# gunrock/mini

Measured on AMD Instinct MI355X. Metric: MTEPS (million traversed edges/sec) BFS advance+filter, RMAT-22, higher is better.
Workload: dtype int32

## Files before the change

### include/mgx/bfs_fused.hpp

```cpp
#pragma once
#include <cstdlib>
#include <cstring>
#include <memory>

#include "runtime.hpp"
#include "env.hpp"
#include "wave.hpp"

namespace mgx {

constexpr int BFS_MAX_TRACE = 4096;
constexpr int BFS_VSHIFT = 38;
constexpr u64 BFS_EMASK = (1ull << BFS_VSHIFT) - 1ull;

struct bfs_ctrl_t {
  u64 cursor[3];
  u64 pad_a_[13];
  u64 lcursor[3];
  u64 pad_b_[13];
  u64 ledges[3];
  u64 pad_c_[13];
  u64 reached;
  u64 pad_d_[15];
  u64 merged_new;
// ... 64 lines not shown
  const int* ub_col;
  const u32* ub_col24;
  const int* ub_owner;
  u32 ub_units;
  u32 ub_units_pad;
  u32 ub_hot_only;
  const u32* ubf_col24;
  const int* ubf_owner;
  u32 ubf_units_pad;
  u32 dense_div;
  u32 vs_v[4];
  u32 vs_v9;
  u32 vs_edges;
  u32 vs_div;
  u32 vs_dummy;
  u32* flush_buf;
  u32 defer_min_marks;
  u32 defer_words;
  u32 defer_reach_mul, defer_reach_div;
  int lazy_pull;
  int merged_pull;
  u32 chain_max_edges;
  u32 chain_big_edges;
  u32 lazy_div;
  u32* slot_marks;
  const int* cold_owner;
  const int* cold_dst;
  int cold_slices;
  u32 cold_lo[BFS_COLD_MAX_SLICES];
  u32 cold_off[BFS_COLD_MAX_SLICES + 1];
// ... 793 lines not shown
  int src_plan = 1;
  int defer_words = -1;
  int defer_mul = 1, defer_div = 1;
  int do_chain = 1;
  int merged_pull = 1;
  int seed_chain = 1;
  int tail_chain = 1;
  int tail_front = 1;
  int chain_big = -1;
  int cold = 1;
  int lazy = -1;
  long long defer = -1;
  int spin = -1;
  int build_list = 0;
  int mini = 1;
  int batch_overlap = 1;
  int many_spare = 0;
#ifdef MGX_LAB
  int flags = 0;
  int build_diag = 0;
  int dense_diag = 0;
#endif
  static bfs_run_opts_t from_env() {
    bfs_run_opts_t o;
    auto geti = [](const char* name, int& out) { if (const char* e = mgx::env(name)) out = atoi(e); };
    auto getll = [](const char* name, long long& out) { if (const char* e = mgx::env(name)) out = atoll(e); };
    geti("MGX_BFS_COLD_TEST", o.cold_test);
    geti("MGX_BFS_MERGED_PUSH", o.merged);
    geti("MGX_BFS_DENSE", o.dense);
    geti("MGX_BFS_VSHORT", o.vshort);
// ... 7 lines not shown
    geti("MGX_BFS_HOT_UNITS", o.hot_units);
    geti("MGX_BFS_COLD", o.cold);
    if (const char* e = mgx::env("MGX_BFS_DEFER_REACH")) {
      o.defer_mul = atoi(e);
      const char* sl = strchr(e, '/');
      o.defer_div = sl ? atoi(sl + 1) : 1;
      if (o.defer_div < 1) o.defer_div = 1;
    }
    geti("MGX_BFS_SEED_CHAIN", o.seed_chain);
    geti("MGX_BFS_MERGED_PULL", o.merged_pull);
    geti("MGX_BFS_DO_CHAIN", o.do_chain);
    geti("MGX_BFS_TAIL_CHAIN", o.tail_chain);
    geti("MGX_BFS_TAIL_FRONT", o.tail_front);
    geti("MGX_BFS_CHAIN_BIG_EDGES", o.chain_big);
    geti("MGX_BFS_MINI", o.mini);
    geti("MGX_BFS_BATCH_OVERLAP", o.batch_overlap);
    if (o.many_spare < 0) o.many_spare = 0;
    geti("MGX_BFS_LAZY", o.lazy);
    if (o.lazy > (1 << 20)) o.lazy = 1 << 20;
#ifdef MGX_LAB
    geti("MGX_BFS_FLAGS", o.flags);
    geti("MGX_BFS_BUILD_DIAG", o.build_diag);
    geti("MGX_BFS_DENSE_DIAG", o.dense_diag);
#else
#endif
    return o;
  }
};

struct bfs_alt_state_t {
// ... 108 lines not shown
```

### include/mgx/bfs_fused_mini.hpp

```cpp
#pragma once
#include "bfs_fused.hpp"
#include "bfs_fused_chain.hpp"

namespace mgx {

constexpr int BFS_MINI_WGS = 64;
constexpr int BFS_MINI_LCAP = 4096;
constexpr int BFS_MINI_WCAP = 8192;
constexpr u32 BFS_MINI_EDGES_LATE = 131072;
constexpr u32 BFS_MINI_EDGES_EARLY = 32768;
constexpr u32 BFS_MINI_SHORT_ROWS = 65536;
constexpr size_t bfs_mini_lds_bytes() {
  return (size_t)(2 * BFS_MINI_LCAP + 4) * 4 + (size_t)BFS_MINI_WCAP * 4 + 64 * 8 + 256;
}

__device__ __forceinline__ bool bfs_level_is_mini(const bfs_fused_args_t& a, const bfs_ctrl_t* c, int slot) {
  if (a.mode != 0 || c->lazy_slot == slot) return false;
  const u64 cur = c->cursor[slot % 3], lcur = c->lcursor[slot % 3];
  const u64 E = (cur & BFS_EMASK) + c->ledges[slot % 3];
  const bool late = c->reached * 4ull >= (u64)(u32)a.n;
  return (lcur >> BFS_VSHIFT) <= (u64)BFS_MINI_LCAP && (cur >> BFS_VSHIFT) <= (u64)BFS_MINI_SHORT_ROWS &&
         E <= (u64)(late ? BFS_MINI_EDGES_LATE : BFS_MINI_EDGES_EARLY);
}

template <int NT>
__device__ __forceinline__ void bfs_mini_body(const bfs_fused_args_t& a, int arg, u32 blk, u32 nblk) {
  constexpr int NW = NT / WAVE;
  constexpr u64 CNT1 = 1ull << 40;
  constexpr u64 DEGMASK = CNT1 - 1ull;
  extern __shared__ __attribute__((aligned(16))) char smem[];
  u32* const s_loff = (u32*)smem;
  u32* const s_lrow = s_loff + BFS_MINI_LCAP + 4;
  u32* const s_win = s_lrow + BFS_MINI_LCAP;
  u64* const s_scan = (u64*)(s_win + BFS_MINI_WCAP);
  __shared__ int s_cnt, s_maxdeg;
  __shared__ u64 s_base[2];
  __shared__ u32 s_long_true;
  bfs_ctrl_t* const c = a.ctrl;
  int slot, level;
  bfs_resolve(c, arg, slot, level);
  if (c->done) return;
  const u64 cur = c->cursor[slot % 3], lcur = c->lcursor[slot % 3];
  const u64 ledges = c->ledges[slot % 3];
  const int nf_s = (int)(cur >> BFS_VSHIFT), nf_l = (int)(lcur >> BFS_VSHIFT);
  const u32 Es = (u32)(cur & BFS_EMASK), Rl = (u32)(lcur & BFS_EMASK);
  const int in = slot & 1, out = (slot + 1) & 1;
  const bool first_thread = blk == 0 && threadIdx.x == 0;
  if (nf_s + nf_l == 0) {
    if (first_thread) {
      c->cursor[(slot + 2) % 3] = 0; c->lcursor[(slot + 2) % 3] = 0; c->ledges[(slot + 2) % 3] = 0;
// ... 37 lines not shown
    c->sum_long_vertices += (u64)nf_l;
    c->push_levels += 1;
    c->small_levels += 1;
    c->mini_slots += 1;
    c->slots += 1;
    c->slot_level[(slot + 1) & 3] = level + 1;
    c->flush_count[(slot + 1) & 1] = 0;
    bfs_slot_marks_clear(a, slot + 1);
    c->fb_slot = -1;
  }
  const int lane = lane_id();
  const int wave = threadIdx.x / WAVE;
  const u32 long_min = a.long_min > 0 ? (u32)a.long_min : 0xFFFFFFFFu;
  const int new_label = level + 1;
  for (int i = threadIdx.x; i < nf_l; i += NT) { s_loff[i] = a.lq_off[in][i]; s_lrow[i] = a.lq_row[in][i]; }
  if (threadIdx.x == 0) { s_loff[nf_l] = Rl; s_cnt = 0; s_maxdeg = 0; }
  __syncthreads();

  u64* const cur_s = &c->cursor[(slot + 1) % 3];
  u64* const cur_l = &c->lcursor[(slot + 1) % 3];
  u32* __restrict__ const out_row_s = a.fr_row[out];
  u32* __restrict__ const out_off_s = a.fr_off[out];
  u32* __restrict__ const out_row_l = a.lq_row[out];
  u32* __restrict__ const out_off_l = a.lq_off[out];
  int found = 0;

  auto flush = [&]() {
    __syncthreads();
    const int W = s_cnt;
    for (int first = 0; first < W; first += NT) {
      const int i = first + (int)threadIdx.x;
// ... 20 lines not shown
        if (tot_l >> 40) atomicAdd(&c->ledges[(slot + 1) % 3], (u64)s_long_true);
      }
      __syncthreads();
      if (deg) {
        const u64 b = is_long ? s_base[1] : s_base[0];
        const u64 at = is_long ? ex_l : ex_s;
        const u64 pos = (b >> BFS_VSHIFT) + (at >> 40);
        (is_long ? out_row_l : out_row_s)[pos] = ro;
        (is_long ? out_off_l : out_off_s)[pos] = (u32)((b & BFS_EMASK) + (at & DEGMASK)) | (is_long ? (deg & 63u) : 0u);
      }
      __syncthreads();
    }
    if (threadIdx.x == 0) s_cnt = 0;
    __syncthreads();
  };
  auto visit = [&](bool act, u32 d) {
    bool win = false;
    if (act) {
      const u32 bit = 1u << (d & 31u);
      const u32 seen = a.visited[d >> 5];
      if (!(seen & bit)) win = !(atomicOr(a.visited + (d >> 5), bit) & bit);
    }
    const u64 bal = __ballot(win);
    if (bal) {
      int at = 0;
      if (lane == 0) at = atomicAdd(&s_cnt, __popcll(bal));
      at = __builtin_amdgcn_readfirstlane(at);
      if (win) { s_win[at + rank_in_mask(bal)] = d; ++found; }
    }
  };

  {
    const u32 U = Rl >> 6;
    const u32 Wt = nblk * NW, w0 = blk * NW + (u32)wave;
    const u32 iters = (U + Wt - 1u) / Wt;
    for (u32 t = 0; t < iters; ++t) {
      const u32 u = w0 + t * Wt;
      bool act = false;
      u32 d = 0;
      if (u < U) {
        const u32 r0 = u << 6;
        int lo = 0, hi = nf_l;
        while (hi - lo > 1) { const int mid = (lo + hi) >> 1; if ((s_loff[mid] & ~63u) <= r0) lo = mid; else hi = mid; }
        const u32 e0 = s_loff[lo];
        const u32 deg = bfs_lq_degree(e0, s_loff[lo + 1]);
        const u32 rank = r0 - (e0 & ~63u) + (u32)lane;
        act = rank < deg;
        if (act) d = (u32)a.col_indices[s_lrow[lo] + rank];
      }
      visit(act, d);
      __syncthreads();
      const int cnt_now = s_cnt;
      __syncthreads();
      if (cnt_now > BFS_MINI_WCAP - NT) flush();
    }
  }
  if (nf_s > 0 && (u64)Es >= 4ull * (u64)nf_s) {
    const u32* __restrict__ fr_row = a.fr_row[in];
    const u32* __restrict__ fr_off = a.fr_off[in];
    const u32 iters = (Es + (u32)gthreads - 1u) / (u32)gthreads;
    for (u32 t = 0; t < iters; ++t) {
      const u64 r64 = (u64)gtid + (u64)t * (u64)gthreads;
      const bool act = r64 < (u64)Es;
      const u32 r = act ? (u32)r64 : 0u;
      int lo = 0, hi = nf_s;
      while (hi - lo > 1) { const int mid = (lo + hi) >> 1; if (fr_off[mid] <= r) lo = mid; else hi = mid; }
      const u32 d = act ? (u32)a.col_indices[fr_row[lo] + (r - fr_off[lo])] : 0u;
      visit(act, d);
      __syncthreads();
      const int cnt_now = s_cnt;
      __syncthreads();
      if (cnt_now > BFS_MINI_WCAP - NT) flush();
    }
  } else
  {
    const u32* __restrict__ fr_row = a.fr_row[in];
    const u32* __restrict__ fr_off = a.fr_off[in];
    const u32 iters = ((u32)nf_s + (u32)gthreads - 1u) / (u32)gthreads;
    for (u32 t = 0; t < iters; ++t) {
      const long long i = gtid + (long long)t * gthreads;
      u32 row = 0, deg = 0;
      if (i < nf_s) {
        const u32 e0 = fr_off[i], e1 = (i + 1 < nf_s) ? fr_off[i + 1] : Es;
        row = fr_row[i];
        deg = e1 - e0;
      }
      int wmax = (int)deg;
#pragma unroll
      for (int sh = WAVE / 2; sh > 0; sh >>= 1) { const int o = __shfl_xor(wmax, sh, WAVE); wmax = o > wmax ? o : wmax; }
      if (lane == 0 && wmax) atomicMax(&s_maxdeg, wmax);
      __syncthreads();
      const u32 kmax = (u32)s_maxdeg;
      for (u32 k = 0; k < kmax; ++k) {
        const bool act = k < deg;
        const u32 d = act ? (u32)a.col_indices[row + k] : 0u;
        visit(act, d);
        __syncthreads();
        const int cnt_now = s_cnt;
        __syncthreads();
        if (cnt_now > BFS_MINI_WCAP - NT) flush();
      }
      __syncthreads();
      if (threadIdx.x == 0) s_maxdeg = 0;
      __syncthreads();
    }
  }
  flush();
  found = (int)wave_sum((u32)found);
  if (lane == 0 && found) atomicAdd(&c->reached_mini, (u64)found);
}
template <int NT>
__global__ __launch_bounds__(NT) void k_bfs_mini(bfs_fused_args_t a, int arg) {
  bfs_mini_body<NT>(a, arg, blockIdx.x, gridDim.x);
}

}
```

### include/mgx/bfs_fused_run.hpp

```cpp
#pragma once
#include <cassert>
#include <cstring>
#include <vector>
#include <unistd.h>
#include "bfs_fused.hpp"
#include "bfs_fused_chain.hpp"
#include "bfs_fused_cold.hpp"
#include "bfs_fused_dense.hpp"
#include "bfs_fused_mini.hpp"
#include "bfs_fused_pull.hpp"
#include "bfs_fused_stream.hpp"
#include "bfs_fused_vshort.hpp"
#include "bfs_fused_sparse.hpp"
#include "bfs_fused_wave.hpp"
#include "row_layout.hpp"

namespace mgx {

struct bfs_layout_t {
  const int* row_offsets = nullptr;
  const int* col_indices = nullptr;
  const int* new_of_old = nullptr;
  const int* old_of_new = nullptr;
  const row_layout_t* rows = nullptr;
// ... 108 lines not shown
  if (c->lazy_slot == slot) return;
  if (!bfs_level_is_chained(a, cur, lcur, c->ledges[slot % 3], a.chain_big_edges, BFS_CHAIN_CAP_BIG)) return;
  bfs_chain_body<1024, true, BFS_CHAIN_CAP_BIG>(a, slot, level);
}
__global__ __launch_bounds__(1024) void k_bfs_chain_inplace(bfs_fused_args_t a, int arg) {
  bfs_chain_inplace_body(a, arg);
}

struct bfs_seam_init_t {
  long long nwords;
  const bfs_ctrl_t* prev_ctrl;
  bfs_ctrl_t* prev_head;
  int src, head_words;
};
static_assert(2 * sizeof(bfs_fused_args_t) + sizeof(bfs_seam_init_t) + 64 <= 4096, "a seam launch's two argument structs fit the 4 KB of kernel arguments");
__global__ __launch_bounds__(1024) void k_bfs_seam_mini_init(bfs_fused_args_t a, int arg_a, bfs_fused_args_t b, bfs_seam_init_t init) {
  if (blockIdx.x < (u32)BFS_MINI_WGS) bfs_mini_body<1024>(a, arg_a, blockIdx.x, (u32)BFS_MINI_WGS);
  else bfs_init_body<1024>(b, init.src, init.nwords, init.prev_ctrl, init.prev_head, init.head_words, blockIdx.x - (u32)BFS_MINI_WGS,
                           gridDim.x - (u32)BFS_MINI_WGS);
}
__global__ __launch_bounds__(1024) void k_bfs_seam_chain_chain(bfs_fused_args_t a, int arg_a, bfs_fused_args_t b, int arg_b) {
  if (blockIdx.x == 0) bfs_chain_inplace_body(a, arg_a);
  else bfs_chain_inplace_body(b, arg_b);
}
__global__ __launch_bounds__(1024) void k_bfs_seam_chain_init(bfs_fused_args_t a, int arg_a, bfs_fused_args_t b, bfs_seam_init_t init) {
  if (blockIdx.x == 0) bfs_chain_inplace_body(a, arg_a);
  else bfs_init_body<1024>(b, init.src, init.nwords, init.prev_ctrl, init.prev_head, init.head_words, blockIdx.x - 1u, gridDim.x - 1u);
}

#ifdef MGX_LAB
__global__ __launch_bounds__(1024, 8) void k_bfs_push_stream_diag(bfs_fused_args_t a, int arg) {
  const bfs_slot_plan_t p = bfs_slot_plan(a, arg);
  if (p.empty || p.chained) return;
  bfs_stream_body<1024, BFS_STREAM_HOTW2, 8, false, true, true>(a, p.slot, blockIdx.x, gridDim.x, p.level);
// ... 74 lines not shown
inline void bfs_launch_push(const bfs_fused_args_t& a, int level, standard_context_t& ctx, int open_here, bool coldt, u32 grid_div = 1) {
  if (grid_div < 1u) grid_div = 1u;
  u32 per = (u32)ctx.num_cus * 2 / grid_div;
  if (per < 32u) per = 32u;
  const u32 nstream = a.long_min > 0 ? per : 0u;
  const u32 nwave = per;
  const u32 ncold = a.cold_dst ? a.cold_wgs[a.cold_slices] : 0u;
  if (coldt) hipLaunchKernelGGL(k_bfs_push_level<true>, dim3(ncold + nstream + nwave), dim3(1024), bfs_push_lds_bytes(), ctx.stream(), a, level, nstream, open_here, ncold);
  else hipLaunchKernelGGL(k_bfs_push_level<false>, dim3(ncold + nstream + nwave), dim3(1024), bfs_push_lds_bytes(), ctx.stream(), a, level, nstream, open_here, ncold);
}

struct bfs_launch_plan_t {
  bfs_fused_args_t a;
  bool coldt = false, build2_ok = false;
  bool minis = false;
  u32 nstream = 0, nwave = 0, ncold = 0;
  int lab_flags = 0;
  long long nwords = 0;
  int mode = 0;
  int* labels = nullptr;
};

inline bfs_launch_plan_t bfs_fused_plan(bfs_fused_state_t& st, const int* row_offsets, const int* col_indices, int* labels,
                                        standard_context_t& ctx, const bfs_layout_t* layout, int mode, float alpha,
                                        const int* in_offsets, const int* in_indices) {
  bfs_launch_plan_t plan;
  bfs_fused_args_t& a = plan.a;
  const bfs_run_opts_t& opt = st.opts;
  const bool relabelled = layout && layout->row_offsets;
  static const row_layout_t no_rows;
// ... 51 lines not shown
    a.ub_col24 = R.ubh.col24.data(); a.ub_owner = R.ubh.owner.data();
    a.ub_units = (u32)R.ubh.units; a.ub_units_pad = (u32)R.ubh.units_pad;
  }
  a.ub_hot_only = hot_units ? 1u : 0u;
  a.ubf_col24 = hot_units ? R.ub.col24.data() : nullptr; a.ubf_owner = hot_units ? R.ub.owner.data() : nullptr;
  a.ubf_units_pad = hot_units ? (u32)R.ub.units_pad : 0u;
  const bool packed = units && st.opts.pack24 && (R.ub.col24.data() != nullptr || hot_units);
  a.dense_div = !units ? 0u : (opt.dense >= 0 ? (u32)opt.dense : (packed ? 8u : st.dense_div));
  const bool vs = relabelled && R.vs_dummy != 0 && R.vs_long_min == st.long_min && st.long_min > 0 && !coldt && !lab_flags &&
                  R.vs_edges > 0;
  for (int i = 0; i < 4; ++i) a.vs_v[i] = vs ? R.vs_v[i] : 0u;
  a.vs_v9 = (vs && R.vs_v9 >= R.vs_v[1] && R.vs_v9 <= R.vs_v[2]) ? R.vs_v9 : (vs ? R.vs_v[2] : 0u);
  a.vs_edges = vs ? R.vs_edges : 0u;
  a.vs_dummy = vs ? R.vs_dummy : 0u;
  a.vs_div = !vs ? 0u : (opt.vshort >= 0 ? (u32)opt.vshort : st.vshort_div);
#ifdef MGX_LAB
  a.dense_diag = opt.dense_diag;
  a.build_diag = opt.build_diag;
#endif
  if (!st.slot_marks.size()) st.slot_marks = mem_t<u32>((size_t)2 * BFS_MARK_CTRS * BFS_MARK_STRIDE, ctx);
  a.slot_marks = st.slot_marks.data();
  a.merged_pull = (mode == 1 && opt.merged_pull && opt.merged && !lab_flags) ? 1 : 0;
  const long long defer = opt.defer >= 0 ? opt.defer : (long long)st.defer_min_marks;
  if (defer > 0 && !lab_flags && !st.flush_buf.size()) st.flush_buf = mem_t<u32>((size_t)BFS_FLUSH_MAX * BFS_FLUSH_WORDS, ctx);
  a.flush_buf = (defer > 0 && !lab_flags) ? st.flush_buf.data() : nullptr;
  a.defer_min_marks = (u32)defer;
  {
    int dw = opt.defer_words >= 0 ? opt.defer_words : BFS_FLUSH_WORDS;
    if (dw > BFS_FLUSH_WORDS) dw = BFS_FLUSH_WORDS;
    a.defer_words = (u32)(dw / 32 * 32);
// ... 14 lines not shown
  for (int i = 0; i <= BFS_COLD_MAX_SLICES; ++i) a.cold_cb[i] = cold_pk ? R.cold_cb[i] : 0u;
  for (int i = 0; i < BFS_COLD_MAX_SLICES; ++i) a.cold_lo[i] = cold ? R.cold_lo[i] : 0u;
  for (int i = 0; i <= BFS_COLD_MAX_SLICES; ++i) { a.cold_off[i] = cold ? R.cold_off[i] : 0u; a.cold_wgs[i] = cold ? R.cold_wgs[i] : 0u; }
  const bool colds = cold && a.vs_div && R.colds_pairs > 0 && R.colds_dst.data() && opt.cold != 2;
  a.colds_owner = colds ? R.colds_owner.data() : nullptr;
  a.colds_dst = colds ? R.colds_dst.data() : nullptr;
  for (int i = 0; i <= BFS_COLD_MAX_SLICES; ++i) a.colds_off[i] = colds ? R.colds_off[i] : 0u;
  const size_t cold_words = cold ? (size_t)R.cold_wgs[R.cold_slices] * BFS_COLD_WORDS : 0;
  if (cold && st.cold_flush.size() < cold_words) { ctx.synchronize(); st.cold_flush = mem_t<u32>(cold_words, ctx); }
  a.cold_flush = cold ? st.cold_flush.data() : nullptr;
  a.lazy_pull = (mode == 1 && build2_ok && !opt.build_list && opt.lazy != 0) ? 1 : 0;
  a.lazy_div = (a.dense_div && a.vs_div && build2_ok && !opt.build_list && !a.cold_all) ? (opt.lazy >= 0 ? (u32)opt.lazy : st.lazy_div) : 0u;
  plan.coldt = coldt;
  plan.build2_ok = build2_ok;
  plan.minis = mode == 0 && opt.mini != 0 && a.chain_big_edges != 0u && opt.merged && !lab_flags && (st.n >= (1 << 22) || opt.mini == 2);
  plan.nstream = a.long_min > 0 ? (u32)ctx.num_cus * 2 : 0u;
  plan.nwave = (u32)ctx.num_cus * 2;
  plan.ncold = (!coldt && a.cold_dst) ? a.cold_wgs[a.cold_slices] : 0u;
  plan.lab_flags = lab_flags;
  plan.nwords = nwords;
  plan.mode = mode;
  plan.labels = labels;
  return plan;
}

inline bool bfs_wants_src_shapes(const bfs_fused_state_t& st, int mode) {
  return mode == 0 && st.opts.src_plan && st.opts.tail_chain && st.opts.mini != 0 && st.opts.merged && st.opts.seed_chain &&
         (st.n >= (1 << 22) || st.opts.mini == 2);
}
inline int bfs_classify_source(const bfs_fused_state_t& st, const bfs_launch_plan_t& plan, const bfs_layout_t* layout, int src, int idx = 0) {
// ... 3 lines not shown
  const unsigned* const sh = layout->src_shapes + (size_t)idx * 4;
  const u64 deg = sh[0], e1 = sh[1], s1 = sh[2], l1 = sh[3];
  if (deg == 0 || e1 == 0xFFFFFFFFull) return BFS_SRC_UNKNOWN;
  if ((1ull + s1 + l1) * 4ull >= (u64)(u32)a.n) return BFS_SRC_UNKNOWN;
  const u64 lim = a.chain_big_edges < BFS_CHAIN_EARLY_EDGES ? a.chain_big_edges : BFS_CHAIN_EARLY_EDGES;
  const u64 chain_cap = lim < (u64)BFS_CHAIN_CAP_BIG ? lim : (u64)BFS_CHAIN_CAP_BIG;
  u64 E, rs, rl;
  if (deg > chain_cap) {
    const bool is_long = a.long_min > 0 && deg >= (u64)a.long_min;
    E = deg; rs = is_long ? 0 : 1; rl = is_long ? 1 : 0;
  } else if (e1 > chain_cap) {
    E = e1; rs = s1; rl = l1;
  } else {
    return BFS_SRC_UNKNOWN;
  }
  const bool mini = rl <= (u64)BFS_MINI_LCAP && rs <= (u64)BFS_MINI_SHORT_ROWS && E <= (u64)BFS_MINI_EDGES_EARLY;
  return mini ? BFS_SRC_ABSORB : BFS_SRC_SKIP;
}
inline int bfs_class_slots(const bfs_fused_state_t& st, int cls) {
  if (cls == BFS_SRC_UNKNOWN) return st.slots_hint;
  if (st.cls_at[cls] > 0) return st.cls_max[cls];
  if (cls == BFS_SRC_SKIP && st.cls_at[BFS_SRC_ABSORB] > 0) return st.cls_max[BFS_SRC_ABSORB] + 1 > st.slots_hint ? st.cls_max[BFS_SRC_ABSORB] + 1 : st.slots_hint;
  return st.slots_hint;
}

inline void bfs_enqueue_chain_inplace(const bfs_launch_plan_t& plan, int slot, hipStream_t s) {
  hipLaunchKernelGGL(k_bfs_chain_inplace, dim3(1), dim3(1024), bfs_chain_lds_bytes(BFS_CHAIN_CAP_BIG), s, plan.a, bfs_slot_arg(slot));
}
inline void bfs_enqueue_mini(const bfs_launch_plan_t& plan, int slot, hipStream_t s) {
  hipLaunchKernelGGL(k_bfs_mini<1024>, dim3(BFS_MINI_WGS), dim3(1024), bfs_mini_lds_bytes(), s, plan.a, bfs_slot_arg(slot));
}
inline int bfs_enqueue_start(const bfs_fused_state_t& st, const bfs_launch_plan_t& plan, int src, standard_context_t& ctx,
                             const bfs_ctrl_t* prev_ctrl = nullptr, bfs_ctrl_t* prev_head = nullptr, int head_words = 0,
                             bool front_mini = true) {
  hipStream_t s = ctx.stream();
  hipLaunchKernelGGL(k_bfs_fused_init, dim3(grid_for(((long long)st.n + 3) / 4, BLOCK, ctx.num_cus * 8)), dim3(BLOCK), 0, s, plan.a, src,
                     plan.nwords, prev_ctrl, prev_head, head_words);
  if (plan.a.chain_big_edges) bfs_enqueue_chain_inplace(plan, 0, s);
  if (plan.minis && front_mini) { bfs_enqueue_mini(plan, 0, s); return 1; }
  return 0;
}
inline bool bfs_fused_plan_alt(bfs_fused_state_t& st, const bfs_launch_plan_t& plan, standard_context_t& ctx, bfs_launch_plan_t& p) {
  if (!st.alt && !st.alt_refused) {
    st.alt = bfs_alt_state_t::make(st.n, st.bitmap_words(), ctx);
    st.alt_refused = !st.alt;
// ... 13 lines not shown
  a.ctrl = t.ctrl;
  a.slot_marks = t.slot_marks;
  return true;
}
inline void bfs_enqueue_seam(const bfs_fused_state_t& st, const bfs_launch_plan_t& plan_a, const bfs_launch_plan_t& tail_a, int sl_a,
                             const bfs_launch_plan_t& plan_b, int src, bfs_ctrl_t* prev_head, int head_words, standard_context_t& ctx) {
  hipStream_t s = ctx.stream();
  bfs_seam_init_t init;
  init.nwords = plan_b.nwords;
  init.prev_ctrl = plan_b.a.ctrl;
  init.prev_head = prev_head;
  init.src = src;
  init.head_words = head_words;
  const int want = grid_for(((long long)st.n + 3) / 4, 1024, 1 << 20);
  if (plan_a.minis) {
    int ninit = ctx.num_cus - BFS_MINI_WGS;
    if (ninit < 64) ninit = 64;
    if (ninit > want) ninit = want;
    hipLaunchKernelGGL(k_bfs_seam_mini_init, dim3(BFS_MINI_WGS + ninit), dim3(1024), bfs_mini_lds_bytes(), s, plan_a.a, bfs_slot_arg(sl_a),
                       plan_b.a, init);
    hipLaunchKernelGGL(k_bfs_seam_chain_chain, dim3(2), dim3(1024), bfs_chain_lds_bytes(BFS_CHAIN_CAP_BIG), s, tail_a.a, bfs_slot_arg(sl_a + 1),
                       plan_b.a, bfs_slot_arg(0));
  } else {
    int ninit = ctx.num_cus - 1;
    if (ninit < 16) ninit = 16;
    if (ninit > want) ninit = want;
    hipLaunchKernelGGL(k_bfs_seam_chain_init, dim3(1 + ninit), dim3(1024), bfs_chain_lds_bytes(BFS_CHAIN_CAP_BIG), s, tail_a.a, bfs_slot_arg(sl_a),
                       plan_b.a, init);
    bfs_enqueue_chain_inplace(plan_b, 0, s);
  }
}
inline void bfs_enqueue_build(const bfs_fused_state_t& st, const bfs_launch_plan_t& plan, int arg, hipStream_t s) {
  if (st.opts.build_list || !plan.build2_ok)
    hipLaunchKernelGGL((k_bfs_build<512, true>), dim3(bfs_build_grid(st.n, 512)), dim3(512), 0, s, plan.a, arg,
                       (const u32*)nullptr, plan.labels, st.n, 1, 0, 1);
// ... 17 lines not shown
  st.tail_from = 1 << 30;
  if (!(a.chain_big_edges && st.opts.tail_chain)) return;
  const int lv = hc->levels < trace_avail ? hc->levels : trace_avail;
  int kind[64];
  const int L = lv < 64 ? lv : 64;
  bool pulled = false;
  u64 reached = 1;
  int extra_big = lv > 64 ? lv - 64 : 0;
  (void)extra_big;
  for (int l = 0; l < L; ++l) {
    const u64 t = hc->trace[l];
    if (l > 0) reached += t >> BFS_VSHIFT;
    const bool late = reached * 4ull >= (u64)(u32)a.n;
    const u64 lim = late || a.chain_big_edges < BFS_CHAIN_EARLY_EDGES ? a.chain_big_edges : BFS_CHAIN_EARLY_EDGES;
    bool small = (t >> BFS_VSHIFT) <= (u64)BFS_CHAIN_CAP_BIG && (t & BFS_EMASK) <= lim;
    bool mid = (t >> BFS_VSHIFT) <= (u64)BFS_MINI_SHORT_ROWS && (t & BFS_EMASK) <= (u64)(late ? BFS_MINI_EDGES_LATE : BFS_MINI_EDGES_EARLY);
    if (mode == 1) {
      const float unvisited = (float)((long long)a.n - (long long)reached);
      if (unvisited < (float)(long long)(t >> BFS_VSHIFT) * a.alpha) pulled = true;
      if (pulled) small = false;
      mid = false;
    }
    kind[l] = small ? 0 : (minis && mid ? 1 : 2);
  }
  auto slots_needed = [&](bool front_mini) {
    int lo = 0, hi = L;
    while (lo < hi && kind[lo] == 0) ++lo;
    if (minis && front_mini && lo < hi && kind[lo] == 1) ++lo;
    while (hi > lo && kind[hi - 1] == 0) --hi;
    if (minis && hi > lo && kind[hi - 1] == 1) {
      --hi;
// ... 64 lines not shown
          else
#endif
          bfs_launch_push_part<2>(a, arg, ctx, coldt, nstream + ncold, nstream);
        }
        if (timed) MGX_HIP(hipEventRecord(st.wev[3 * i + 1], s));
        bfs_launch_push_part<3>(a, arg, ctx, coldt, nwave, 0);
        if (timed) MGX_HIP(hipEventRecord(st.wev[3 * i + 2], s));
      } else {
        bfs_launch_push_part<0>(a, arg, ctx, coldt, nstream + ncold + nwave, nstream);
      }
      if (mode == 1 && !a.merged_pull)
        hipLaunchKernelGGL(k_bfs_pull_level<256>, dim3(ctx.num_cus * 8), dim3(256), 0, s, a, arg);
      bfs_enqueue_build(st, plan, arg, s);
      if (timed_merged) MGX_HIP(hipEventRecord(st.wev[3 * i + 2], s));
    }
    if (plan.minis && batch == 0) { bfs_enqueue_mini(plan, slot, s); ++slot; }
    if (a.chain_big_edges && (slot >= st.tail_from || plan.minis) && opt.tail_chain) chain_inplace(slot);
    if (batch_events) MGX_HIP(hipEventRecord(st.ev1, s));
    constexpr size_t head_bytes = offsetof(bfs_ctrl_t, trace) + 64 * sizeof(u64);
    if ((opt.spin >= 0 ? opt.spin != 0 : st.spin) && !batch_events) {
      const u64 seq = ++st.seq;
      hipLaunchKernelGGL(k_bfs_publish, dim3(1), dim3(256), 0, s, (const bfs_ctrl_t*)st.ctrl.data(), st.host_ctrl.data(), st.host_seq.data(), seq,
                         (int)(head_bytes / 4));
      MGX_CHECK_LAUNCH("fused BFS: kernel launch");
      volatile u64* const flag = st.host_seq.data();
      long long spins = 0;
      while (*flag != seq) {
        if (++spins > 20000000LL) { MGX_HIP(hipStreamSynchronize(s)); break; }
        __builtin_ia32_pause();
      }
      __atomic_thread_fence(__ATOMIC_ACQUIRE);
// ... 106 lines not shown
    const bfs_launch_plan_t& P = plans[me];
    bfs_ctrl_t* const prev_head = pending[me] >= 0 ? bfs_many_head(heads, pending[me]) : (bfs_ctrl_t*)nullptr;
    pending[me] = i;
    int sl;
    if (i == 0 || state_of(i - 1) == me) {
      sl = bfs_enqueue_start(st, P, srcs[i], ctx, prev_head ? P.a.ctrl : (const bfs_ctrl_t*)nullptr, prev_head, head_words, cls != BFS_SRC_SKIP);
    } else {
      const int sl_a = plan.minis ? last_slots[(size_t)i - 1] - 1 : last_slots[(size_t)i - 1];
      bfs_enqueue_seam(st, plans[me ^ 1], tails[me ^ 1], sl_a, P, srcs[i], prev_head, head_words, ctx);
      sl = 0;
      if (plan.minis && cls != BFS_SRC_SKIP) { bfs_enqueue_mini(P, 0, s); sl = 1; }
    }
    for (int k = 0; k < my_slots; ++k, ++sl) bfs_enqueue_slot(st, P, sl, ctx);
    if (overlap && i + 1 == lead && !st.alt) second_state();
    const bool seam_behind = i + 1 < count && state_of(i + 1) != me;
    if (plan.minis) { if (!seam_behind) bfs_enqueue_mini(P, sl, s); ++sl; }
    if (tail && !seam_behind) bfs_enqueue_chain_inplace(tails[me], sl, s);
    last_slots[(size_t)i] = sl;
    classes[(size_t)i] = cls;
  }
  tail_guard.release();
  const u64 seq = ++st.seq;
  assert(pending[0] == count - 1);
  if (pending[1] >= 0)
    hipLaunchKernelGGL(k_bfs_publish2, dim3(1), dim3(256), 0, s, (const bfs_ctrl_t*)plans[0].a.ctrl, bfs_many_head(heads, pending[0]),
                       (const bfs_ctrl_t*)plans[1].a.ctrl, bfs_many_head(heads, pending[1]), st.host_seq.data(), seq, head_words);
  else
    hipLaunchKernelGGL(k_bfs_publish, dim3(1), dim3(256), 0, s, (const bfs_ctrl_t*)st.ctrl.data(), bfs_many_head(heads, count - 1), st.host_seq.data(), seq, head_words);
  MGX_CHECK_LAUNCH("fused BFS (batch of sources): kernel launch");
  {
    volatile u64* const flag = st.host_seq.data();
// ... 31 lines not shown
```

### include/mgx/env.hpp

```cpp
#pragma once
#include <cstdio>
#include <cstdlib>
#include <cstring>

namespace mgx {

struct env_switch_t { const char* name; const char* what; };

inline const env_switch_t* env_switches(int* count) {
  static const env_switch_t table[] = {
    {"MGX_BFS_DENSE", "0 / N: unit-block body for long rows off / a level takes it from frontier edges >= units / N"},
    {"MGX_BFS_VSHORT", "0 / N: short rows vertex by vertex off / threshold divisor"},
    {"MGX_BFS_LAZY", "0 / N: lazy queues off / the build writes no queues behind a push that stored >= n / N marks"},
    {"MGX_BFS_COLD", "0 / 2 (lab: 1): cold-edge pass off / on"},
    {"MGX_BFS_COLD_LISTS", "0 / 1 (lab: 2): whether the layout builds the long rows' cold-edge lists"},
    {"MGX_BFS_COLD_PACK", "0: keep the 8-byte cold pairs instead of the packed 4-byte ones"},
    {"MGX_BFS_COLD_TEST", "0 / 1: bitmap probe of cold neighbours off / on (default: by graph size)"},
    {"MGX_BFS_FLAT_LISTS", "0: a flat graph keeps the ordinary layout instead of all-entry pair lists"},
    {"MGX_BFS_HOT_UNITS", "0: no second copy of the unit blocks without the cold lists' entries"},
    {"MGX_BFS_PACK24", "0: 32-bit unit-block entries instead of the 24-bit copy"},
    {"MGX_BFS_MINI", "0 / 2: no M launches / M launches on every graph (default: from 2^22 vertices on)"},
    {"MGX_BFS_BATCH_OVERLAP", "0: a batch of sources runs in one traversal state, no launch shared by two traversals"},
    {"MGX_BFS_SEED_CHAIN", "0: the chain of small levels at the start runs inside slot 0's push launch"},
    {"MGX_BFS_TAIL_CHAIN", "0: no in-place chain launch behind the last slots"},
    {"MGX_BFS_TAIL_FRONT", "0: no chain in front of the last slots"},
    {"MGX_BFS_CHAIN_BIG_EDGES", "largest level an in-place chain launch runs (edges)"},
    {"MGX_BFS_CHAIN_MAX_EDGES", "largest level block 0 runs inside the push launch (0: no chains)"},
    {"MGX_BFS_MERGED_PUSH", "0: the parts of a slot's push as separate launches"},
    {"MGX_BFS_MERGED_PULL", "0: direction-optimising runs: the bottom-up sweep as a launch of its own"},
    {"MGX_BFS_DO_CHAIN", "0: direction-optimising runs: no chains of small top-down levels"},
    {"MGX_BFS_DEFER", "0 / N: deferred hot marks off / a workgroup flushes its bitmap above N claims"},
    {"MGX_BFS_DEFER_REACH", "\"mul/div\": a level defers its hot marks while reached * mul < range * div"},
    {"MGX_BFS_DEFER_WORDS", "words of the bitmap prefix whose marks are deferred (default: all)"},
    {"MGX_BFS_BUILD_LIST", "1: the list-based queue build of round 1"},
    {"MGX_BFS_SRC_PLAN", "0: no per-source launch plan"},
    {"MGX_BFS_LONG_MIN", "long-row threshold of the layout (entries)"},
// ... 58 lines not shown
```

Baseline: 462,700.

## Widen mini BFS launch for late levels and restage short-row expansion in LDS

Adds a late-level rule that sends levels behind the peak with up to a configurable edge count (default 1M) into the mini kernel. When it applies, the tail launch and the seam init launch are sized to the CU count instead of 64 workgroups. The short-row expansion now gives each workgroup a contiguous edge share and stages the row offsets in LDS in chunks, replacing the per-thread global binary search and the degree-max loop. It also halves the window capacity, drops per-iteration barriers in favour of periodic flushes, and issues relaxed atomic loads with batched visited reads. This trades possible lost occupancy or imbalance for fewer launches and less synchronisation on tail levels.

```diff
diff --git a/include/mgx/bfs_fused.hpp b/include/mgx/bfs_fused.hpp
--- a/include/mgx/bfs_fused.hpp
+++ b/include/mgx/bfs_fused.hpp
@@ -102,6 +102,7 @@
   u32 vs_edges;
   u32 vs_div;
   u32 vs_dummy;
+  u32 mini_late_edges;
   u32* flush_buf;
   u32 defer_min_marks;
   u32 defer_words;
@@ -925,6 +926,7 @@
   int spin = -1;
   int build_list = 0;
   int mini = 1;
+  int mini_late_edges = -1;
   int batch_overlap = 1;
   int many_spare = 0;
 #ifdef MGX_LAB
@@ -962,6 +964,7 @@
     geti("MGX_BFS_TAIL_FRONT", o.tail_front);
     geti("MGX_BFS_CHAIN_BIG_EDGES", o.chain_big);
     geti("MGX_BFS_MINI", o.mini);
+    geti("MGX_BFS_MINI_LATE_EDGES", o.mini_late_edges);
     geti("MGX_BFS_BATCH_OVERLAP", o.batch_overlap);
     if (o.many_spare < 0) o.many_spare = 0;
     geti("MGX_BFS_LAZY", o.lazy);
diff --git a/include/mgx/bfs_fused_mini.hpp b/include/mgx/bfs_fused_mini.hpp
--- a/include/mgx/bfs_fused_mini.hpp
+++ b/include/mgx/bfs_fused_mini.hpp
@@ -6,21 +6,39 @@
 
 constexpr int BFS_MINI_WGS = 64;
 constexpr int BFS_MINI_LCAP = 4096;
-constexpr int BFS_MINI_WCAP = 8192;
+constexpr int BFS_MINI_WCAP = 4096;
 constexpr u32 BFS_MINI_EDGES_LATE = 131072;
 constexpr u32 BFS_MINI_EDGES_EARLY = 32768;
 constexpr u32 BFS_MINI_SHORT_ROWS = 65536;
+constexpr u32 BFS_MINI_LATE_EDGES_DEFAULT = 1u << 20;
+constexpr u32 BFS_MINI_LATE_FINDS = 131072;
 constexpr size_t bfs_mini_lds_bytes() {
   return (size_t)(2 * BFS_MINI_LCAP + 4) * 4 + (size_t)BFS_MINI_WCAP * 4 + 64 * 8 + 256;
+}
+static_assert(bfs_mini_lds_bytes() <= 64 * 1024, "an init workgroup fits beside an M workgroup on a CU");
+
+__host__ __device__ constexpr bool bfs_mini_takes(u64 rows_s, u64 rows_l, u64 E, u64 reached, u32 n, u32 vs3, u32 late_edges) {
+  if (rows_l > (u64)BFS_MINI_LCAP) return false;
+  const bool late = reached * 4ull >= (u64)n;
+  if (!late) return rows_s <= (u64)BFS_MINI_SHORT_ROWS && E <= (u64)BFS_MINI_EDGES_EARLY;
+  if (vs3 == 0u || late_edges <= BFS_MINI_EDGES_LATE) return rows_s <= (u64)BFS_MINI_SHORT_ROWS && E <= (u64)BFS_MINI_EDGES_LATE;
+  const u64 finds = (u64)vs3 > reached ? (u64)vs3 - reached : 0ull;
+  return E <= (u64)late_edges && finds <= (u64)BFS_MINI_LATE_FINDS;
+}
+inline int bfs_mini_tail_wgs(u32 late_edges, int num_cus) {
+  if (late_edges <= BFS_MINI_EDGES_LATE) return BFS_MINI_WGS;
+  return num_cus > 0 ? num_cus : 1;
 }
 
 __device__ __forceinline__ bool bfs_level_is_mini(const bfs_fused_args_t& a, const bfs_ctrl_t* c, int slot) {
   if (a.mode != 0 || c->lazy_slot == slot) return false;
   const u64 cur = c->cursor[slot % 3], lcur = c->lcursor[slot % 3];
   const u64 E = (cur & BFS_EMASK) + c->ledges[slot % 3];
-  const bool late = c->reached * 4ull >= (u64)(u32)a.n;
-  return (lcur >> BFS_VSHIFT) <= (u64)BFS_MINI_LCAP && (cur >> BFS_VSHIFT) <= (u64)BFS_MINI_SHORT_ROWS &&
-         E <= (u64)(late ? BFS_MINI_EDGES_LATE : BFS_MINI_EDGES_EARLY);
+  return bfs_mini_takes(cur >> BFS_VSHIFT, lcur >> BFS_VSHIFT, E, c->reached, (u32)a.n, a.vs_v[3], a.mini_late_edges);
+}
+template <typename V>
+__device__ __forceinline__ V bfs_mini_load(const V* p) {
+  return __hip_atomic_load(p, __ATOMIC_RELAXED, __HIP_MEMORY_SCOPE_WAVEFRONT);
 }
 
 template <int NT>
@@ -33,7 +51,7 @@
   u32* const s_lrow = s_loff + BFS_MINI_LCAP + 4;
   u32* const s_win = s_lrow + BFS_MINI_LCAP;
   u64* const s_scan = (u64*)(s_win + BFS_MINI_WCAP);
-  __shared__ int s_cnt, s_maxdeg;
+  __shared__ int s_cnt;
   __shared__ u64 s_base[2];
   __shared__ u32 s_long_true;
   bfs_ctrl_t* const c = a.ctrl;
@@ -101,7 +119,7 @@
   const u32 long_min = a.long_min > 0 ? (u32)a.long_min : 0xFFFFFFFFu;
   const int new_label = level + 1;
   for (int i = threadIdx.x; i < nf_l; i += NT) { s_loff[i] = a.lq_off[in][i]; s_lrow[i] = a.lq_row[in][i]; }
-  if (threadIdx.x == 0) { s_loff[nf_l] = Rl; s_cnt = 0; s_maxdeg = 0; }
+  if (threadIdx.x == 0) { s_loff[nf_l] = Rl; s_cnt = 0; }
   __syncthreads();
 
   u64* const cur_s = &c->cursor[(slot + 1) % 3];
@@ -152,13 +170,10 @@
     if (threadIdx.x == 0) s_cnt = 0;
     __syncthreads();
   };
-  auto visit = [&](bool act, u32 d) {
+  auto claim = [&](bool act, u32 d, u32 seen) {
     bool win = false;
-    if (act) {
-      const u32 bit = 1u << (d & 31u);
-      const u32 seen = a.visited[d >> 5];
-      if (!(seen & bit)) win = !(atomicOr(a.visited + (d >> 5), bit) & bit);
-    }
+    const u32 bit = 1u << (d & 31u);
+    if (act && !(seen & bit)) win = !(atomicOr(a.visited + (d >> 5), bit) & bit);
     const u64 bal = __ballot(win);
     if (bal) {
       int at = 0;
@@ -168,14 +183,16 @@
     }
   };
 
-  {
+  if (nf_l > 0) {
+    constexpr u32 PERIOD = (u32)(BFS_MINI_WCAP / NT);
+    static_assert(BFS_MINI_WCAP % NT == 0 && BFS_MINI_WCAP >= NT, "whole steps of the workgroup between two flushes");
     const u32 U = Rl >> 6;
     const u32 Wt = nblk * NW, w0 = blk * NW + (u32)wave;
     const u32 iters = (U + Wt - 1u) / Wt;
     for (u32 t = 0; t < iters; ++t) {
       const u32 u = w0 + t * Wt;
       bool act = false;
-      u32 d = 0;
+      u32 at = 0;
       if (u < U) {
         const u32 r0 = u << 6;
         int lo = 0, hi = nf_l;
@@ -184,66 +201,68 @@
         const u32 deg = bfs_lq_degree(e0, s_loff[lo + 1]);
         const u32 rank = r0 - (e0 & ~63u) + (u32)lane;
         act = rank < deg;
-        if (act) d = (u32)a.col_indices[s_lrow[lo] + rank];
-      }
-      visit(act, d);
-      __syncthreads();
-      const int cnt_now = s_cnt;
-      __syncthreads();
-      if (cnt_now > BFS_MINI_WCAP - NT) flush();
-    }
-  }
-  if (nf_s > 0 && (u64)Es >= 4ull * (u64)nf_s) {
+        at = s_lrow[lo] + (act ? rank : 0u);
+      } else {
+        at = s_lrow[0];
+      }
+      const u32 d = (u32)bfs_mini_load(a.col_indices + at);
+      const u32 seen = bfs_mini_load(a.visited + (d >> 5));
+      claim(act, d, seen);
+      if ((t + 1u) % PERIOD == 0u && t + 1u < iters) flush();
+    }
+    flush();
+  }
+  if (nf_s > 0) {
+    constexpr int PER = BFS_MINI_WCAP / NT;
+    u32* const s_off = (u32*)smem;
+    u32* const s_row = s_off + BFS_MINI_WCAP + 4;
+    static_assert(BFS_MINI_WCAP <= BFS_MINI_LCAP, "the short rows' stage fits where the long-row queue was");
     const u32* __restrict__ fr_row = a.fr_row[in];
     const u32* __restrict__ fr_off = a.fr_off[in];
-    const u32 iters = (Es + (u32)gthreads - 1u) / (u32)gthreads;
-    for (u32 t = 0; t < iters; ++t) {
-      const u64 r64 = (u64)gtid + (u64)t * (u64)gthreads;
-      const bool act = r64 < (u64)Es;
-      const u32 r = act ? (u32)r64 : 0u;
-      int lo = 0, hi = nf_s;
-      while (hi - lo > 1) { const int mid = (lo + hi) >> 1; if (fr_off[mid] <= r) lo = mid; else hi = mid; }
-      const u32 d = act ? (u32)a.col_indices[fr_row[lo] + (r - fr_off[lo])] : 0u;
-      visit(act, d);
-      __syncthreads();
-      const int cnt_now = s_cnt;
-      __syncthreads();
-      if (cnt_now > BFS_MINI_WCAP - NT) flush();
-    }
-  } else
-  {
-    const u32* __restrict__ fr_row = a.fr_row[in];
-    const u32* __restrict__ fr_off = a.fr_off[in];
-    const u32 iters = ((u32)nf_s + (u32)gthreads - 1u) / (u32)gthreads;
-    for (u32 t = 0; t < iters; ++t) {
-      const long long i = gtid + (long long)t * gthreads;
-      u32 row = 0, deg = 0;
-      if (i < nf_s) {
-        const u32 e0 = fr_off[i], e1 = (i + 1 < nf_s) ? fr_off[i + 1] : Es;
-        row = fr_row[i];
-        deg = e1 - e0;
-      }
-      int wmax = (int)deg;
-#pragma unroll
-      for (int sh = WAVE / 2; sh > 0; sh >>= 1) { const int o = __shfl_xor(wmax, sh, WAVE); wmax = o > wmax ? o : wmax; }
-      if (lane == 0 && wmax) atomicMax(&s_maxdeg, wmax);
-      __syncthreads();
-      const u32 kmax = (u32)s_maxdeg;
-      for (u32 k = 0; k < kmax; ++k) {
-        const bool act = k < deg;
-        const u32 d = act ? (u32)a.col_indices[row + k] : 0u;
-        visit(act, d);
-        __syncthreads();
-        const int cnt_now = s_cnt;
-        __syncthreads();
-        if (cnt_now > BFS_MINI_WCAP - NT) flush();
-      }
-      __syncthreads();
-      if (threadIdx.x == 0) s_maxdeg = 0;
-      __syncthreads();
-    }
-  }
-  flush();
+    const u32 S = (Es + nblk - 1u) / nblk;
+    const u32 nchunks = (S + (u32)BFS_MINI_WCAP - 1u) / (u32)BFS_MINI_WCAP;
+    const u64 share0 = (u64)blk * S;
+    const u32 share1 = (u32)(share0 + S < (u64)Es ? share0 + S : (u64)Es);
+    for (u32 ch = 0; ch < nchunks; ++ch) {
+      const u64 r0_64 = share0 + (u64)ch * BFS_MINI_WCAP;
+      if (r0_64 >= (u64)share1) break;
+      const u32 r0 = (u32)r0_64;
+      const u32 r1 = share1 - r0 > (u32)BFS_MINI_WCAP ? r0 + (u32)BFS_MINI_WCAP : share1;
+      const u32 i0 = (u32)wave_upper_bound(fr_off, (long long)nf_s, r0) - 1u;
+      const u32 cnt = (r1 - r0) < (u32)nf_s - i0 ? (r1 - r0) : (u32)nf_s - i0;
+      for (u32 k = threadIdx.x; k <= cnt; k += NT) {
+        const bool in_q = i0 + k < (u32)nf_s;
+        s_off[k] = in_q ? fr_off[i0 + k] : Es;
+        if (k < cnt) s_row[k] = fr_row[i0 + k];
+      }
+      __syncthreads();
+      const u32 top = 1u << (31 - __clz((int)cnt));
+      u32 pos[PER], rr[PER];
+      bool act[PER];
+#pragma unroll
+      for (int q = 0; q < PER; ++q) {
+        const u32 r = r0 + (u32)q * NT + threadIdx.x;
+        act[q] = r < r1;
+        rr[q] = act[q] ? r : r0;
+        pos[q] = 0u;
+      }
+      for (u32 step = top; step; step >>= 1) {
+#pragma unroll
+        for (int q = 0; q < PER; ++q) {
+          const u32 nx = pos[q] + step;
+          if (nx < cnt && s_off[nx] <= rr[q]) pos[q] = nx;
+        }
+      }
+      u32 d[PER], seen[PER];
+#pragma unroll
+      for (int q = 0; q < PER; ++q) d[q] = (u32)bfs_mini_load(a.col_indices + (s_row[pos[q]] + (rr[q] - s_off[pos[q]])));
+#pragma unroll
+      for (int q = 0; q < PER; ++q) seen[q] = bfs_mini_load(a.visited + (d[q] >> 5));
+#pragma unroll
+      for (int q = 0; q < PER; ++q) claim(act[q], d[q], seen[q]);
+      flush();
+    }
+  }
   found = (int)wave_sum((u32)found);
   if (lane == 0 && found) atomicAdd(&c->reached_mini, (u64)found);
 }
diff --git a/include/mgx/bfs_fused_run.hpp b/include/mgx/bfs_fused_run.hpp
--- a/include/mgx/bfs_fused_run.hpp
+++ b/include/mgx/bfs_fused_run.hpp
@@ -146,10 +146,9 @@
   int src, head_words;
 };
 static_assert(2 * sizeof(bfs_fused_args_t) + sizeof(bfs_seam_init_t) + 64 <= 4096, "a seam launch's two argument structs fit the 4 KB of kernel arguments");
-__global__ __launch_bounds__(1024) void k_bfs_seam_mini_init(bfs_fused_args_t a, int arg_a, bfs_fused_args_t b, bfs_seam_init_t init) {
-  if (blockIdx.x < (u32)BFS_MINI_WGS) bfs_mini_body<1024>(a, arg_a, blockIdx.x, (u32)BFS_MINI_WGS);
-  else bfs_init_body<1024>(b, init.src, init.nwords, init.prev_ctrl, init.prev_head, init.head_words, blockIdx.x - (u32)BFS_MINI_WGS,
-                           gridDim.x - (u32)BFS_MINI_WGS);
+__global__ __launch_bounds__(1024, 8) void k_bfs_seam_mini_init(bfs_fused_args_t a, int arg_a, bfs_fused_args_t b, bfs_seam_init_t init, u32 nmini) {
+  if (blockIdx.x < nmini) bfs_mini_body<1024>(a, arg_a, blockIdx.x, nmini);
+  else bfs_init_body<1024>(b, init.src, init.nwords, init.prev_ctrl, init.prev_head, init.head_words, blockIdx.x - nmini, gridDim.x - nmini);
 }
 __global__ __launch_bounds__(1024) void k_bfs_seam_chain_chain(bfs_fused_args_t a, int arg_a, bfs_fused_args_t b, int arg_b) {
   if (blockIdx.x == 0) bfs_chain_inplace_body(a, arg_a);
@@ -254,6 +253,7 @@
   bfs_fused_args_t a;
   bool coldt = false, build2_ok = false;
   bool minis = false;
+  int mini_tail_wgs = BFS_MINI_WGS;
   u32 nstream = 0, nwave = 0, ncold = 0;
   int lab_flags = 0;
   long long nwords = 0;
@@ -335,6 +335,7 @@
   a.vs_edges = vs ? R.vs_edges : 0u;
   a.vs_dummy = vs ? R.vs_dummy : 0u;
   a.vs_div = !vs ? 0u : (opt.vshort >= 0 ? (u32)opt.vshort : st.vshort_div);
+  a.mini_late_edges = opt.mini_late_edges >= 0 ? (u32)opt.mini_late_edges : BFS_MINI_LATE_EDGES_DEFAULT;
 #ifdef MGX_LAB
   a.dense_diag = opt.dense_diag;
   a.build_diag = opt.build_diag;
@@ -379,6 +380,7 @@
   plan.coldt = coldt;
   plan.build2_ok = build2_ok;
   plan.minis = mode == 0 && opt.mini != 0 && a.chain_big_edges != 0u && opt.merged && !lab_flags && (st.n >= (1 << 22) || opt.mini == 2);
+  plan.mini_tail_wgs = bfs_mini_tail_wgs(a.mini_late_edges, ctx.num_cus);
   plan.nstream = a.long_min > 0 ? (u32)ctx.num_cus * 2 : 0u;
   plan.nwave = (u32)ctx.num_cus * 2;
   plan.ncold = (!coldt && a.cold_dst) ? a.cold_wgs[a.cold_slices] : 0u;
@@ -412,7 +414,7 @@
   } else {
     return BFS_SRC_UNKNOWN;
   }
-  const bool mini = rl <= (u64)BFS_MINI_LCAP && rs <= (u64)BFS_MINI_SHORT_ROWS && E <= (u64)BFS_MINI_EDGES_EARLY;
+  const bool mini = bfs_mini_takes(rs, rl, E, 0ull, (u32)a.n, a.vs_v[3], a.mini_late_edges);
   return mini ? BFS_SRC_ABSORB : BFS_SRC_SKIP;
 }
 inline int bfs_class_slots(const bfs_fused_state_t& st, int cls) {
@@ -425,8 +427,8 @@
 inline void bfs_enqueue_chain_inplace(const bfs_launch_plan_t& plan, int slot, hipStream_t s) {
   hipLaunchKernelGGL(k_bfs_chain_inplace, dim3(1), dim3(1024), bfs_chain_lds_bytes(BFS_CHAIN_CAP_BIG), s, plan.a, bfs_slot_arg(slot));
 }
-inline void bfs_enqueue_mini(const bfs_launch_plan_t& plan, int slot, hipStream_t s) {
-  hipLaunchKernelGGL(k_bfs_mini<1024>, dim3(BFS_MINI_WGS), dim3(1024), bfs_mini_lds_bytes(), s, plan.a, bfs_slot_arg(slot));
+inline void bfs_enqueue_mini(const bfs_launch_plan_t& plan, int slot, hipStream_t s, bool tail = false) {
+  hipLaunchKernelGGL(k_bfs_mini<1024>, dim3(tail ? plan.mini_tail_wgs : BFS_MINI_WGS), dim3(1024), bfs_mini_lds_bytes(), s, plan.a, bfs_slot_arg(slot));
 }
 inline int bfs_enqueue_start(const bfs_fused_state_t& st, const bfs_launch_plan_t& plan, int src, standard_context_t& ctx,
                              const bfs_ctrl_t* prev_ctrl = nullptr, bfs_ctrl_t* prev_head = nullptr, int head_words = 0,
@@ -470,11 +472,12 @@
   init.head_words = head_words;
   const int want = grid_for(((long long)st.n + 3) / 4, 1024, 1 << 20);
   if (plan_a.minis) {
-    int ninit = ctx.num_cus - BFS_MINI_WGS;
+    const int nmini = plan_a.mini_tail_wgs;
+    int ninit = nmini > BFS_MINI_WGS ? ctx.num_cus : ctx.num_cus - BFS_MINI_WGS;
     if (ninit < 64) ninit = 64;
     if (ninit > want) ninit = want;
-    hipLaunchKernelGGL(k_bfs_seam_mini_init, dim3(BFS_MINI_WGS + ninit), dim3(1024), bfs_mini_lds_bytes(), s, plan_a.a, bfs_slot_arg(sl_a),
-                       plan_b.a, init);
+    hipLaunchKernelGGL(k_bfs_seam_mini_init, dim3(nmini + ninit), dim3(1024), bfs_mini_lds_bytes(), s, plan_a.a, bfs_slot_arg(sl_a),
+                       plan_b.a, init, (u32)nmini);
     hipLaunchKernelGGL(k_bfs_seam_chain_chain, dim3(2), dim3(1024), bfs_chain_lds_bytes(BFS_CHAIN_CAP_BIG), s, tail_a.a, bfs_slot_arg(sl_a + 1),
                        plan_b.a, bfs_slot_arg(0));
   } else {
@@ -522,7 +525,7 @@
     const bool late = reached * 4ull >= (u64)(u32)a.n;
     const u64 lim = late || a.chain_big_edges < BFS_CHAIN_EARLY_EDGES ? a.chain_big_edges : BFS_CHAIN_EARLY_EDGES;
     bool small = (t >> BFS_VSHIFT) <= (u64)BFS_CHAIN_CAP_BIG && (t & BFS_EMASK) <= lim;
-    bool mid = (t >> BFS_VSHIFT) <= (u64)BFS_MINI_SHORT_ROWS && (t & BFS_EMASK) <= (u64)(late ? BFS_MINI_EDGES_LATE : BFS_MINI_EDGES_EARLY);
+    bool mid = bfs_mini_takes(t >> BFS_VSHIFT, 0ull, t & BFS_EMASK, reached, (u32)a.n, a.vs_v[3], a.mini_late_edges);
     if (mode == 1) {
       const float unvisited = (float)((long long)a.n - (long long)reached);
       if (unvisited < (float)(long long)(t >> BFS_VSHIFT) * a.alpha) pulled = true;
@@ -617,7 +620,7 @@
       bfs_enqueue_build(st, plan, arg, s);
       if (timed_merged) MGX_HIP(hipEventRecord(st.wev[3 * i + 2], s));
     }
-    if (plan.minis && batch == 0) { bfs_enqueue_mini(plan, slot, s); ++slot; }
+    if (plan.minis && batch == 0) { bfs_enqueue_mini(plan, slot, s, true); ++slot; }
     if (a.chain_big_edges && (slot >= st.tail_from || plan.minis) && opt.tail_chain) chain_inplace(slot);
     if (batch_events) MGX_HIP(hipEventRecord(st.ev1, s));
     constexpr size_t head_bytes = offsetof(bfs_ctrl_t, trace) + 64 * sizeof(u64);
@@ -754,7 +757,7 @@
     for (int k = 0; k < my_slots; ++k, ++sl) bfs_enqueue_slot(st, P, sl, ctx);
     if (overlap && i + 1 == lead && !st.alt) second_state();
     const bool seam_behind = i + 1 < count && state_of(i + 1) != me;
-    if (plan.minis) { if (!seam_behind) bfs_enqueue_mini(P, sl, s); ++sl; }
+    if (plan.minis) { if (!seam_behind) bfs_enqueue_mini(P, sl, s, true); ++sl; }
     if (tail && !seam_behind) bfs_enqueue_chain_inplace(tails[me], sl, s);
     last_slots[(size_t)i] = sl;
     classes[(size_t)i] = cls;
diff --git a/include/mgx/env.hpp b/include/mgx/env.hpp
--- a/include/mgx/env.hpp
+++ b/include/mgx/env.hpp
@@ -20,6 +20,7 @@
     {"MGX_BFS_HOT_UNITS", "0: no second copy of the unit blocks without the cold lists' entries"},
     {"MGX_BFS_PACK24", "0: 32-bit unit-block entries instead of the 24-bit copy"},
     {"MGX_BFS_MINI", "0 / 2: no M launches / M launches on every graph (default: from 2^22 vertices on)"},
+    {"MGX_BFS_MINI_LATE_EDGES", "largest level behind the peak (edges) an M launch takes on a layout; 131072: the old rule and 64-workgroup launch"},
     {"MGX_BFS_BATCH_OVERLAP", "0: a batch of sources runs in one traversal state, no launch shared by two traversals"},
     {"MGX_BFS_SEED_CHAIN", "0: the chain of small levels at the start runs inside slot 0's push launch"},
     {"MGX_BFS_TAIL_CHAIN", "0: no in-place chain launch behind the last slots"},
```

Result: slower. 439,500 (-5.0%).
